# spkelle2/simple_mip_solver

Hardware: NVIDIA B200
Metric: node_lp_solves_per_sec (higher is better)
Workload: dtype f64

## Files before the change

### simple_mip_solver_b200/csrc/blp.cu

```cuda
#include "../../include/blp.h"

#include <cuda_runtime.h>
#include <dlfcn.h>

#include <cstdarg>
#include <cstdio>
#include <cstdlib>
#include <cstring>
#include <string>
#include <vector>

#include "blp_kernels.cuh"
#include "blp_prep.hpp"
#include "blp_simplex.cuh"

using namespace blp;

namespace {

thread_local std::string g_err;

int fail(int code, const char* fmt, ...) {
    char buf[512];
    va_list ap;
// ... 618 lines not shown
    return (o && o->max_active > 0 && o->max_active < B) ? o->max_active : B;
}

int blp_ld(int B) { return B <= 0 ? 0 : (B + kBlk - 1) / kBlk * kBlk; }

const char* blp_last_error(void) { return g_err.c_str(); }

const char* blp_version(void) {
#ifdef BLP_TUNING
    return "blp 0.2 sm_100a (tuning build: BLP_* environment variables are read)";
#else
    return "blp 0.2 sm_100a";
#endif
}

int blp_create(int device, int m, int n, int64_t nnz, const int32_t* rowptr, const int32_t* colidx,
               const double* val, const double* c, const double* row_lb, blp_handle* out) {
    if (!out) return fail(BLP_ERR_ARG, "blp_create: out is NULL");
    *out = nullptr;
    if (m < 1 || n < 1 || nnz < 0 || !rowptr || !c || !row_lb || (nnz > 0 && (!colidx || !val)))
        return fail(BLP_ERR_ARG, "blp_create: need m >= 1, n >= 1, nnz >= 0 and non-NULL arrays");
    if (rowptr[0] != 0 || rowptr[m] != nnz)
        return fail(BLP_ERR_ARG, "blp_create: rowptr[0] must be 0 and rowptr[m] must equal nnz");
    for (int i = 0; i < m; ++i) {
        if (rowptr[i + 1] < rowptr[i]) return fail(BLP_ERR_ARG, "blp_create: rowptr not monotone at row %d", i);
        if (!(std::fabs(row_lb[i]) < 1e30))
            return fail(BLP_ERR_ARG, "blp_create: row_lb[%d] is not finite (rows are 'a.x >= b')", i);
    }
    for (int64_t p = 0; p < nnz; ++p)
        if (colidx[p] < 0 || colidx[p] >= n || !std::isfinite(val[p]))
            return fail(BLP_ERR_ARG, "blp_create: entry %lld has column %d / non-finite value", (long long)p, colidx[p]);
    for (int j = 0; j < n; ++j)
        if (!std::isfinite(c[j])) return fail(BLP_ERR_ARG, "blp_create: c[%d] is not finite", j);
    int ndev = 0;
    CK(cudaGetDeviceCount(&ndev));
    if (device < 0 || device >= ndev)
        return fail(BLP_ERR_ARG, "blp_create: device %d out of range (%d visible)", device, ndev);
    CK(cudaSetDevice(device));
    blp_handle h = new (std::nothrow) blp_handle_s;
    if (!h) return fail(BLP_ERR_NOMEM, "blp_create: out of host memory");
    h->device = device;
    h->m_base = m;
    h->n = n;
    h->A0.rows = m;
    h->A0.cols = n;
    h->A0.ptr.assign(rowptr, rowptr + m + 1);
    h->A0.idx.assign(colidx, colidx + nnz);
    h->A0.val.assign(val, val + nnz);
    h->c0.assign(c, c + n);
    h->b0.assign(row_lb, row_lb + m);
    cudaDeviceGetAttribute(&h->num_sms, cudaDevAttrMultiProcessorCount, device);
    cudaDeviceGetAttribute(&h->coop_ok, cudaDevAttrCooperativeLaunch, device);
    cudaError_t e = cudaStreamCreateWithFlags(&h->stream, cudaStreamNonBlocking);
    if (e == cudaSuccess) e = cudaFuncSetAttribute(k_primal2<true>, cudaFuncAttributeMaxDynamicSharedMemorySize, 64 * 1024);
    if (e == cudaSuccess) e = cudaFuncSetAttribute(k_primal2<false>, cudaFuncAttributeMaxDynamicSharedMemorySize, 64 * 1024);
    if (e == cudaSuccess) e = cudaFuncSetAttribute(k_dual2<true>, cudaFuncAttributeMaxDynamicSharedMemorySize, 64 * 1024);
    if (e == cudaSuccess) e = cudaFuncSetAttribute(k_dual2<false>, cudaFuncAttributeMaxDynamicSharedMemorySize, 64 * 1024);
    if (e == cudaSuccess) e = cudaMallocHost(&h->h_counters, 16 * sizeof(int32_t));
    for (int q = 0; q < 4 && e == cudaSuccess; ++q) e = cudaEventCreate(&h->ev[q]);
    for (int q = 0; q < blp_handle_s::kLanes - 1 && e == cudaSuccess; ++q) {
        e = cudaStreamCreateWithFlags(&h->side[q], cudaStreamNonBlocking);
        if (e == cudaSuccess) e = cudaEventCreateWithFlags(&h->ev_join[q], cudaEventDisableTiming);
    }
    if (e == cudaSuccess) e = cudaEventCreateWithFlags(&h->ev_fork, cudaEventDisableTiming);
    if (e != cudaSuccess) {
        blp_destroy(h);
        return fail(BLP_ERR_CUDA, "blp_create: %s", cudaGetErrorString(e));
    }
    int rc = prepare(h);
    if (rc != BLP_OK) {
        blp_destroy(h);
        return rc;
    }
    *out = h;
    return BLP_OK;
}

int blp_append_rows(blp_handle h, int k, const int32_t* rowptr, const int32_t* colidx,
                    const double* val, const double* rhs, int* first_row_id) {
    if (!h) return fail(BLP_ERR_ARG, "blp_append_rows: NULL handle");
    if (k < 1 || !rowptr || !rhs) return fail(BLP_ERR_ARG, "blp_append_rows: need k >= 1 rows");
    if (rowptr[0] != 0) return fail(BLP_ERR_ARG, "blp_append_rows: rowptr[0] must be 0");
    const int64_t nnz = rowptr[k];
    for (int i = 0; i < k; ++i) {
        if (rowptr[i + 1] < rowptr[i]) return fail(BLP_ERR_ARG, "blp_append_rows: rowptr not monotone");
        if (!(std::fabs(rhs[i]) < 1e30)) return fail(BLP_ERR_ARG, "blp_append_rows: rhs[%d] not finite", i);
    }
    for (int64_t p = 0; p < nnz; ++p)
        if (colidx[p] < 0 || colidx[p] >= h->n || !std::isfinite(val[p]))
            return fail(BLP_ERR_ARG, "blp_append_rows: bad entry %lld", (long long)p);
    CK(cudaSetDevice(h->device));
    const int first = h->A0.rows;
    const int32_t base = h->A0.ptr.back();
    for (int i = 0; i < k; ++i) h->A0.ptr.push_back(base + rowptr[i + 1]);
    h->A0.idx.insert(h->A0.idx.end(), colidx, colidx + nnz);
    h->A0.val.insert(h->A0.val.end(), val, val + nnz);
    h->b0.insert(h->b0.end(), rhs, rhs + k);
    h->A0.rows += k;
    if (first_row_id) *first_row_id = first;
    return prepare(h);
}

int blp_truncate_rows(blp_handle h, int m_keep) {
    if (!h) return fail(BLP_ERR_ARG, "blp_truncate_rows: NULL handle");
    if (m_keep < h->m_base || m_keep > h->A0.rows)
        return fail(BLP_ERR_ARG, "blp_truncate_rows: m_keep %d outside [%d, %d]", m_keep, h->m_base, h->A0.rows);
    if (m_keep == h->A0.rows) return BLP_OK;
    CK(cudaSetDevice(h->device));
    h->A0.rows = m_keep;
    h->A0.ptr.resize(m_keep + 1);
// ... 70 lines not shown
    CK(cudaEventRecord(h->ev[0], st));
    CK(cudaMemsetAsync(S.counters, 0, 16 * sizeof(int32_t), st));
    if (freeze) CK(cudaMemsetAsync(cfrz_ws, 0, frz_bytes, st));
    if (have_mask)
        CK(cudaMemcpy2DAsync(mask_ws, S.ld, row_mask, ld_in, S.ld, P.m - P.m_base, cudaMemcpyDeviceToDevice, st));
    if (want_frac) {
        CK(cudaMemsetAsync(isint_ws, 0, P.n, st));
        k_set_isint<<<(n_int + 255) / 256, 256, 0, st>>>(int_idx, n_int, P.n, isint_ws);
        ++launches;
    }
    if (x) CK(cudaMemsetAsync(x, 0, (size_t)P.n * ld_in * sizeof(double), st));
    if (y) CK(cudaMemsetAsync(y, 0, (size_t)P.m * ld_in * sizeof(double), st));
    if (ld_in > B) {
        k_out_pad<<<(ld_in - B + 127) / 128, 128, 0, st>>>(O, B, ld_in);
        ++launches;
    }
    k_init_nodes<<<(S.ld + 127) / 128, 128, 0, st>>>(P, S);
    k_init_cols<<<elementwise_grid((size_t)P.n * S.ld), kCtaThreads, 0, st>>>(P, S, lb, ub, x0, ld_in);
    k_init_rows<<<elementwise_grid((size_t)P.m * S.ld), kCtaThreads, 0, st>>>(P, S, y0, ld_in);
    {
        Plan er0 = plan_rows(P.m, W, 1, kEvalChunks);
        er0.NT = NT;
        launch_check_rows(P, S, er0, 0, st);
    }
    k_build_lumask<<<elementwise_grid((size_t)P.n * (S.ld / 32) * 32), kCtaThreads, 0, st>>>(P, S);
    k_count_active<<<(W + 127) / 128, 128, 0, st>>>(S);
    launches += 6;
    CK(cudaGetLastError());
    CK(cudaMemcpyAsync(h->h_counters, S.counters, 13 * sizeof(int32_t), cudaMemcpyDeviceToHost, st));
    CK(cudaStreamSynchronize(st));
    int active = h->h_counters[0];

    auto make_plan = [&](int rows, int width, int rows_per_warp, int max_chunks) {
        Plan p = plan_rows(rows, width, rows_per_warp, max_chunks);
        const int pass = kWarps * (32 / NT);
        p.NT = NT;
        p.tiles = (width + NT - 1) / NT;
        int rpc = pass * std::max(rows_per_warp, 1);
        if (max_chunks > 0) {
            const int need = (rows + max_chunks - 1) / max_chunks;
            rpc = std::max(rpc, ((need + pass - 1) / pass) * pass);
        } else {
            while (rpc > 512 && rpc > pass) rpc -= pass;
        }
        p.rows_per_cta = rpc;
        p.chunks = std::max(1, (rows + rpc - 1) / rpc);
        return p;
    };
    const bool allow_v2 = env_int("BLP_V2", 1) != 0;
    const int graph_lanes = env_int("BLP_GRAPH_LANES", 2);
    const int rpw2 = std::min(env_int("BLP_ROWS_PER_WARP2", 16), kMaxChunkRows / kWarps);
    const int rpw2p = std::min(env_int("BLP_ROWS_PER_WARP2P", freeze ? 24 : rpw2), kMaxChunkRows / kWarps);
    auto step_plan = [&](int rows, int width, bool primal = false) {
        const bool v2 = allow_v2 && width >= kBlk && (long)std::max(P.n, P.m) * width >= (1L << 20);
        int r = v2 ? (primal ? rpw2p : rpw2) : rpw;
        Plan p = make_plan(rows, width, r, 0);
        auto shape = [&](Plan& q, int rr) {
            if (!v2) return;
            q.V = 2;
            q.tiles = (width + kBlk - 1) / kBlk;
            q.rows_per_cta = kWarps * std::max(rr, 1);
            q.chunks = std::max(1, (rows + q.rows_per_cta - 1) / q.rows_per_cta);
        };
        shape(p, r);
        while (r > 1 && (long)p.chunks * p.tiles < 148L * 12) {
            r /= 2;
            p = make_plan(rows, width, r, 0);
            shape(p, r);
        }
        return p;
    };
    Plan pc = step_plan(P.n, W, true), pr = step_plan(P.m, W);
    auto finish_step_plans = [&]() -> int {
        plan_chunks(pc, h->hptrAT, P.n, h->h_chunkC);
        plan_chunks(pr, h->hptrA, P.m, h->h_chunkR);
        CK(upload(h->chunkC, h->h_chunkC, st));
        CK(upload(h->chunkR, h->h_chunkR, st));
        pc.chunk_ptr = h->chunkC.as<int32_t>();
        pr.chunk_ptr = h->chunkR.as<int32_t>();
        return BLP_OK;
    };
    if ((rc = finish_step_plans()) != BLP_OK) return rc;
    Plan ec = make_plan(P.n, W, 1, kEvalChunks), er = make_plan(P.m, W, 1, kEvalChunks);
    D.chunksC = ec.chunks;
    D.chunksR = er.chunks;

    if (active < W) launch_harvest(P, S, O, ec, er, want_frac, st, &launches);

    int next = W, refills = 0;
    auto refill = [&]() -> int {
        while (next < B && active < S.B) {
            const int nnew = std::min(B - next, S.B - active);
            k_refill_plan<<<1, 1024, 0, st>>>(P, S, next, nnew);
            k_refill_cols<<<elementwise_grid((size_t)P.n * nnew), kCtaThreads, 0, st>>>(P, S, lb, ub, x0, ld_in, nnew);
            k_refill_rows<<<elementwise_grid((size_t)P.m * nnew), kCtaThreads, 0, st>>>(P, S, y0, row_mask, ld_in, nnew);
            launch_check_rows(P, S, er, 1, st);
            k_build_lumask<<<elementwise_grid((size_t)P.n * ((S.B + 31) / 32) * 32), kCtaThreads, 0, st>>>(P, S);
            k_count_active<<<(S.B + 127) / 128, 128, 0, st>>>(S);
            launches += 6;
            CK(cudaGetLastError());
            CK(cudaMemcpyAsync(h->h_counters, S.counters, 13 * sizeof(int32_t), cudaMemcpyDeviceToHost, st));
            CK(cudaStreamSynchronize(st));
            next += nnew;
            refills += nnew;
            active = h->h_counters[0];
            if (h->h_counters[3] > 0) launch_harvest(P, S, O, ec, er, want_frac, st, &launches);
        }
        return BLP_OK;
    };
    if ((rc = refill()) != BLP_OK) return rc;
    auto refreeze = [&](int mode) {
        if (!freeze || pc.V != 2) return;
        launches += launch_freeze(P, S, F, T, mode, st);
    };
    refreeze(2);

    const bool profile = o.profile == 1;
    const bool use_graph = o.use_graph && !profile;
    if (profile)
        while ((int)h->prof_ev.size() < 2 * 4 * K0 + 1) {
            cudaEvent_t e;
            CK(cudaEventCreate(&e));
            h->prof_ev.push_back(e);
        }

    bool coop = false;
    bool coop_rejected = false;
    const bool allow_coop = h->coop_ok && env_int("BLP_COOP", 1) != 0;
// ... 818 lines not shown
```

### simple_mip_solver_b200/csrc/blp_kernels.cuh

```cuda
#pragma once
#include <cstdint>
#include <cooperative_groups.h>
#include <cuda_runtime.h>

namespace blp {

#ifndef BLP_U
#define BLP_U 4
#endif
#ifndef BLP_MINB
#define BLP_MINB 6
#endif
#ifndef BLP_ANCHOR32
#define BLP_ANCHOR32 1
#endif
#if BLP_ANCHOR32
using anc_t = float;
using anc2_t = float2;
#else
using anc_t = double;
using anc2_t = double2;
#endif
constexpr int kCtaThreads = 256;
constexpr int kBlk = 64;
// ... 98 lines not shown
            const int4 e = __ldg(reinterpret_cast<const int4*>(ent + p));
            const double v = node_ok ? Vn[(size_t)e.x * ld] : 0.0;
            acc = fma(__hiloint2double(e.w, e.z), v, acc);
        }
    }
    return acc;
}

template <int NT>
__device__ __forceinline__ void row_dot_pair(const int32_t* __restrict__ ptr, const Ent* __restrict__ ent,
                                             int row, bool row_ok, const double* __restrict__ Vn,
                                             const double* __restrict__ Wn, bool node_ok, double& accv,
                                             double& accw) {
    constexpr int ld = kBlk;
    accv = 0.0;
    accw = 0.0;
    if (NT == 32 || (row_ok && node_ok)) {
        const int p0 = __ldg(ptr + row), p1 = __ldg(ptr + row + 1);
        for (int p = p0; p < p1; p += 4) {
            int4 e[4];
            double v[4], w[4];
#pragma unroll
            for (int q = 0; q < 4; ++q) {
                v[q] = 0.0;
                w[q] = 0.0;
                e[q] = make_int4(0, 0, 0, 0);
                if (p + q < p1) {
                    e[q] = __ldg(reinterpret_cast<const int4*>(ent + p + q));
                    if (node_ok) {
                        v[q] = Vn[(size_t)e[q].x * ld];
                        w[q] = Wn[(size_t)e[q].x * ld];
                    }
                }
            }
#pragma unroll
            for (int q = 0; q < 4; ++q) {
                const double cf = __hiloint2double(e[q].w, e[q].z);
                accv = fma(cf, v[q], accv);
                accw = fma(cf, w[q], accw);
            }
        }
    }
}

struct Slab {
    const int* sp;
    const int4* se;
    int base;
    const int* ends = nullptr;
};

extern __shared__ int4 dyn_smem[];

__device__ __forceinline__ Slab stage_slab(const int32_t* __restrict__ ptr,
                                           const Ent* __restrict__ ent, const int r0, const int r1,
                                           const int rows_per_cta, const int cap,
                                           int4* const smem_base = dyn_smem) {
    int* sp = reinterpret_cast<int*>(smem_base);
    int4* se = smem_base + (rows_per_cta + 4) / 4;
    const int nrows = r1 - r0;
    for (int t = threadIdx.x; t <= nrows; t += kCtaThreads) sp[t] = __ldg(ptr + r0 + t);
    __syncthreads();
    Slab s;
    s.sp = sp;
    s.base = sp[0];
    s.se = nullptr;
    const int cnt = sp[nrows] - s.base;
    if (cnt <= cap) {
        const int4* __restrict__ src = reinterpret_cast<const int4*>(ent) + s.base;
        for (int t = threadIdx.x; t < cnt; t += kCtaThreads) se[t] = __ldg(src + t);
        __syncthreads();
        s.se = se;
    }
    return s;
}

template <bool SHARED>
__device__ __forceinline__ double dot_entries(const int4* __restrict__ E, const int p0, const int p1,
                                              const double* __restrict__ Vn, const int ld,
                                              const bool node_ok) {
    constexpr int kU = BLP_U;
    double acc = 0.0;
    for (int p = p0; p < p1; p += kU) {
        double v[kU];
#pragma unroll
        for (int q = 0; q < kU; ++q) {
            v[q] = 0.0;
            if (p + q < p1) {
                const int col = SHARED ? E[p + q].x : __ldg(&E[p + q].x);
                if (node_ok) v[q] = Vn[(size_t)col * ld];
            }
        }
#pragma unroll
        for (int q = 0; q < kU; ++q)
            if (p + q < p1) {
                const int2 c = SHARED ? *reinterpret_cast<const int2*>(&E[p + q].z)
                                      : __ldg(reinterpret_cast<const int2*>(&E[p + q].z));
                acc = fma(__hiloint2double(c.y, c.x), v[q], acc);
            }
    }
    return acc;
}

template <int NT>
__device__ __forceinline__ double slab_dot(const Slab& sl, const Ent* __restrict__ ent, const int lr,
                                           const bool row_ok, const double* __restrict__ Vn,
                                           const int ld, const bool node_ok) {
    if (NT != 32 && !(row_ok && node_ok)) return 0.0;
    const int p0 = sl.sp[lr], p1 = sl.sp[lr + 1];
    if (sl.se) return dot_entries<true>(sl.se - sl.base, p0, p1, Vn, ld, node_ok);
    return dot_entries<false>(reinterpret_cast<const int4*>(ent), p0, p1, Vn, ld, node_ok);
}

constexpr int kLongRow = 96;
// ... 158 lines not shown
    dual_chunk<NT, MAJOR>(P, S, it, rows_per_cta, cap, chunk_ptr, blockIdx.x, blockIdx.y);
}

struct CoopPlan {
    int rpcC, capC, nchC, rpcR, capR, nchR, tiles;
    const int* chunkC;
    const int* chunkR;
};

template <int NT>
__global__ void __launch_bounds__(kCtaThreads, 4)
k_period_coop(const DevProb P, const DevState S, const int K, const CoopPlan C) {
    cooperative_groups::grid_group grid = cooperative_groups::this_grid();
    const int w = blockIdx.x;
    const bool hasC = w < C.nchC * C.tiles, hasR = w < C.nchR * C.tiles;
    const int cxC = w % C.nchC, cyC = w / C.nchC, cxR = w % C.nchR, cyR = w / C.nchR;
    Slab slC{nullptr, nullptr, 0}, slR{nullptr, nullptr, 0};
    int4* const baseR = dyn_smem + (C.rpcC + 4) / 4 + C.capC;
    if (hasC) slC = stage_slab(P.cptr, P.cent, __ldg(C.chunkC + 2 * cxC), __ldg(C.chunkC + 2 * cxC + 1), C.rpcC, C.capC);
    if (hasR) slR = stage_slab(P.rowptr, P.ent, __ldg(C.chunkR + 2 * cxR), __ldg(C.chunkR + 2 * cxR + 1), C.rpcR, C.capR, baseR);
    for (int it = 0; it < K; ++it) {
        const bool major = it == K - 1;
        if (hasC) {
            if (major) primal_chunk<NT, true>(P, S, it, C.rpcC, C.capC, C.chunkC, cxC, cyC, &slC);
            else primal_chunk<NT, false>(P, S, it, C.rpcC, C.capC, C.chunkC, cxC, cyC, &slC);
        }
        grid.sync();
        if (hasR) {
            if (major) dual_chunk<NT, true>(P, S, it, C.rpcR, C.capR, C.chunkR, cxR, cyR, &slR);
            else dual_chunk<NT, false>(P, S, it, C.rpcR, C.capR, C.chunkR, cxR, cyR, &slR);
        }
        grid.sync();
    }
}

#ifndef BLP_MINB2
#define BLP_MINB2 5
#endif

__device__ __forceinline__ double2 ld2(const double* p) { return *reinterpret_cast<const double2*>(p); }
__device__ __forceinline__ double2 ldcs2(const double* p) {
    return __ldcs(reinterpret_cast<const double2*>(p));
}
__device__ __forceinline__ double2 ldcs2(const float* p) {
    const float2 v = __ldcs(reinterpret_cast<const float2*>(p));
    return make_double2((double)v.x, (double)v.y);
}
__device__ __forceinline__ void st2(double* p, const double2 v, const bool k0, const bool k1) {
    if (k0 && k1) *reinterpret_cast<double2*>(p) = v;
    else if (k0) p[0] = v.x;
    else if (k1) p[1] = v.y;
}

template <bool SHARED>
__device__ __forceinline__ void dot2_entries(const int4* __restrict__ E, const int p0, const int p1,
                                             const double* __restrict__ Vn, double& g0, double& g1,
                                             const int ld = kBlk) {
    constexpr int kU = BLP_U;
    for (int p = p0; p < p1; p += kU) {
        double2 v[kU];
#pragma unroll
        for (int q = 0; q < kU; ++q) {
            v[q] = make_double2(0.0, 0.0);
            if (p + q < p1) {
                const int col = SHARED ? E[p + q].x : __ldg(&E[p + q].x);
                v[q] = ld2(Vn + (size_t)col * ld);
            }
        }
#pragma unroll
        for (int q = 0; q < kU; ++q)
            if (p + q < p1) {
                const int2 c = SHARED ? *reinterpret_cast<const int2*>(&E[p + q].z)
                                      : __ldg(reinterpret_cast<const int2*>(&E[p + q].z));
                const double cf = __hiloint2double(c.y, c.x);
                g0 = fma(cf, v[q].x, g0);
                g1 = fma(cf, v[q].y, g1);
            }
    }
}

__device__ __forceinline__ void slab_dot2(const Slab& sl, const Ent* __restrict__ ent, const int lr,
                                          const double* __restrict__ Vn, double& g0, double& g1,
                                          const int ld = kBlk) {
    const int p0 = sl.sp[lr], p1 = sl.ends ? sl.ends[lr] : sl.sp[lr + 1];
    if (sl.se) dot2_entries<true>(sl.se - sl.base, p0, p1, Vn, g0, g1, ld);
    else dot2_entries<false>(reinterpret_cast<const int4*>(ent), p0, p1, Vn, g0, g1, ld);
}


__device__ __forceinline__ void coop_dot2(const Slab& sl, const Ent* __restrict__ ent,
                                          const double* __restrict__ Vn, const int warp, const int lane,
                                          double& g0, double& g1) {
    __shared__ double2 red[kWarps][32];
    const int p0 = sl.sp[0], p1 = sl.ends ? sl.ends[0] : sl.sp[1];
    const int seg = ((p1 - p0 + kWarps - 1) / kWarps + BLP_U - 1) / BLP_U * BLP_U;
    const int a = min(p1, p0 + warp * seg), b = min(p1, a + seg);
    double s0 = 0.0, s1 = 0.0;
    if (sl.se) dot2_entries<true>(sl.se - sl.base, a, b, Vn, s0, s1);
    else dot2_entries<false>(reinterpret_cast<const int4*>(ent), a, b, Vn, s0, s1);
    red[warp][lane] = make_double2(s0, s1);
    __syncthreads();
    g0 = 0.0;
    g1 = 0.0;
#pragma unroll
    for (int w = 0; w < kWarps; ++w) {
        g0 += red[w][lane].x;
        g1 += red[w][lane].y;
    }
}

template <bool SHARED>
__device__ __forceinline__ void dot2_entries_pair(const int4* __restrict__ E, int pa, const int pa1, int pb,
                                                  const int pb1, const double* __restrict__ Vn, double& ga0,
                                                  double& ga1, double& gb0, double& gb1) {
    constexpr int kU = BLP_U;
    while (pa < pa1 || pb < pb1) {
        double2 va[kU], vb[kU];
#pragma unroll
        for (int q = 0; q < kU; ++q) {
            va[q] = make_double2(0.0, 0.0);
            if (pa + q < pa1) {
                const int col = SHARED ? E[pa + q].x : __ldg(&E[pa + q].x);
                va[q] = ld2(Vn + (size_t)col * kBlk);
            }
        }
#pragma unroll
        for (int q = 0; q < kU; ++q) {
            vb[q] = make_double2(0.0, 0.0);
            if (pb + q < pb1) {
                const int col = SHARED ? E[pb + q].x : __ldg(&E[pb + q].x);
                vb[q] = ld2(Vn + (size_t)col * kBlk);
            }
        }
#pragma unroll
        for (int q = 0; q < kU; ++q)
            if (pa + q < pa1) {
                const int2 c = SHARED ? *reinterpret_cast<const int2*>(&E[pa + q].z)
                                      : __ldg(reinterpret_cast<const int2*>(&E[pa + q].z));
                const double cf = __hiloint2double(c.y, c.x);
                ga0 = fma(cf, va[q].x, ga0);
                ga1 = fma(cf, va[q].y, ga1);
            }
#pragma unroll
        for (int q = 0; q < kU; ++q)
            if (pb + q < pb1) {
                const int2 c = SHARED ? *reinterpret_cast<const int2*>(&E[pb + q].z)
                                      : __ldg(reinterpret_cast<const int2*>(&E[pb + q].z));
                const double cf = __hiloint2double(c.y, c.x);
                gb0 = fma(cf, vb[q].x, gb0);
                gb1 = fma(cf, vb[q].y, gb1);
            }
        pa += kU;
        pb += kU;
    }
}

constexpr int kMaxChunkRows = 512;
__shared__ uint16_t s_rows[kMaxChunkRows];
__shared__ int s_ends[kMaxChunkRows];
__shared__ int s_group[kMaxChunkRows / 32 + 1];
__shared__ int s_nrows;

__device__ __forceinline__ Slab stage_slab_frozen(const int32_t* __restrict__ ptr, const Ent* __restrict__ ent,
                                                  const int32_t* __restrict__ ends, const uint8_t* __restrict__ flags,
                                                  const int rows, const int h0, const unsigned live, const int r0,
                                                  const int r1, const int rows_per_cta, const int cap) {
    int* sp = reinterpret_cast<int*>(dyn_smem);
    int4* se = dyn_smem + (rows_per_cta + 4) / 4;
    const int nrows = r1 - r0, lane = threadIdx.x & 31;
    const bool live0 = (live & 0x0000ffffu) != 0, live1 = (live & 0xffff0000u) != 0;
    const uint8_t* __restrict__ f0 = flags + (size_t)h0 * rows + r0;
    const uint8_t* __restrict__ f1 = f0 + rows;
    bool keep[2];
    int rank[2];
#pragma unroll
    for (int q = 0; q < 2; ++q) {
        const int t = threadIdx.x + q * kCtaThreads;
        keep[q] = false;
        if (t <= nrows) sp[t] = __ldg(ptr + r0 + t);
        if (t < nrows) {
            s_ends[t] = __ldg(ends + r0 + t);
            keep[q] = !((!live0 || f0[t] != 0) && (!live1 || f1[t] != 0));
        }
        const unsigned bal = __ballot_sync(0xffffffffu, keep[q]);
        rank[q] = __popc(bal & ((1u << lane) - 1u));
        if (lane == 0) s_group[t >> 5] = __popc(bal);
    }
    __syncthreads();
    Slab s;
    s.sp = sp;
    s.base = sp[0];
    s.se = nullptr;
    s.ends = s_ends;
    const int cnt = sp[nrows] - s.base;
    if (cnt <= cap) {
        const int4* __restrict__ src = reinterpret_cast<const int4*>(ent) + s.base;
        for (int t = threadIdx.x; t < cnt; t += kCtaThreads) se[t] = __ldg(src + t);
        s.se = se;
    }
    const int groups = (nrows + 31) >> 5;
#pragma unroll
    for (int q = 0; q < 2; ++q) {
        const int t = threadIdx.x + q * kCtaThreads;
        if (keep[q]) {
            int before = 0;
            for (int g = 0; g < (t >> 5); ++g) before += s_group[g];
            s_rows[before + rank[q]] = (uint16_t)t;
        }
    }
    if (threadIdx.x == 0) {
        int total = 0;
        for (int g = 0; g < groups; ++g) total += s_group[g];
        s_nrows = total;
    }
    __syncthreads();
    return s;
}

#ifndef BLP_PAIR_ROWS
#define BLP_PAIR_ROWS 0
#endif
#ifndef BLP_PAIR_ROWS_DUAL
#define BLP_PAIR_ROWS_DUAL 0
#endif
#ifndef BLP_MINB2P
#define BLP_MINB2P 4
#endif

template <bool MAJOR>
__global__ void __launch_bounds__(kCtaThreads, BLP_PAIR_ROWS ? BLP_MINB2P : BLP_MINB2)
k_primal2(const DevProb P, const DevState S, const int it, const int rows_per_cta, const int cap,
          const int* __restrict__ chunk_ptr, const int tile0) {
    const int lane = threadIdx.x & 31, warp = threadIdx.x >> 5;
    const int node = (tile0 + blockIdx.y) * kBlk + lane * 2;
    const bool k0 = node < S.B && S.fin[node] == 0;
    const bool k1 = node + 1 < S.B && S.fin[node + 1] == 0;
    const unsigned live = __ballot_sync(0xffffffffu, k0 || k1);
    if (live == 0) return;
    double w0 = 0, w1 = 0, tau0 = 0, tau1 = 0;
    if (k0) {
        const int s = S.sbase[node] + it;
        w0 = (double)s / (double)(s + 1);
        tau0 = S.eta[node] / S.omega[node];
    }
    if (k1) {
        const int s = S.sbase[node + 1] + it;
        w1 = (double)s / (double)(s + 1);
        tau1 = S.eta[node + 1] / S.omega[node + 1];
    }
    const int r0 = __ldg(chunk_ptr + 2 * blockIdx.x);
    const int r1 = __ldg(chunk_ptr + 2 * blockIdx.x + 1);
    const bool frz = !MAJOR && S.cfrz != nullptr;
    const int tile = tile0 + blockIdx.y;
    const Ent* __restrict__ cent = frz ? S.fentAT + (size_t)tile * P.nnz : P.cent;
    const Slab sl = frz ? stage_slab_frozen(P.cptr, cent, S.fendAT + (size_t)tile * P.n, S.cfrz, P.n, tile * 2, live,
                                            r0, r1, rows_per_cta, cap)
                        : stage_slab(P.cptr, P.cent, r0, r1, rows_per_cta, cap);
    const size_t base = tix(0, node, P.n);
    const double* __restrict__ yn = S.y + tix(0, node, P.m);
    const size_t fblk = (size_t)(node >> 5) * P.n;
    const unsigned bit = node & 31;
    const bool coop = (r1 - r0 == 1) && (sl.sp[1] - sl.sp[0] > kLongRow);
    double cg0 = 0.0, cg1 = 0.0;
    if (coop) {
        if (frz && s_nrows == 0) return;
        coop_dot2(sl, cent, yn, warp, lane, cg0, cg1);
        if (warp != 0) return;
    }
#if BLP_PAIR_ROWS
    if (!coop && !frz) {
        for (int j = r0 + warp; j < r1; j += 2 * kWarps) {
            const int jb = j + kWarps;
            const bool hb = jb < r1;
            const size_t ea = base + (size_t)j * kBlk, eb = base + (size_t)(hb ? jb : j) * kBlk;
            const double2 xba = ld2(S.xbar + ea), xbb = ld2(S.xbar + eb);
            const double2 aa = ldcs2(S.xa + ea), ab = ldcs2(S.xa + eb);
            const int jb_ = hb ? jb : j;
            const uint32_t mka = (__ldg(S.lumask + fblk + j) >> bit) & 3u;
            const uint32_t mkb = (__ldg(S.lumask + fblk + jb_) >> bit) & 3u;
            double loa0 = __ldg(S.lref + fblk + j), hia0 = __ldg(S.uref + fblk + j);
            double lob0 = __ldg(S.lref + fblk + jb_), hib0 = __ldg(S.uref + fblk + jb_);
            double loa1 = loa0, hia1 = hia0, lob1 = lob0, hib1 = hib0;
            if (mka) {
                const double2 l2 = ldcs2(S.l + ea), u2 = ldcs2(S.u + ea);
                if (mka & 1u) { loa0 = l2.x; hia0 = u2.x; }
                if (mka & 2u) { loa1 = l2.y; hia1 = u2.y; }
            }
            if (mkb) {
                const double2 l2 = ldcs2(S.l + eb), u2 = ldcs2(S.u + eb);
                if (mkb & 1u) { lob0 = l2.x; hib0 = u2.x; }
                if (mkb & 2u) { lob1 = l2.y; hib1 = u2.y; }
            }
            double ga0 = 0.0, ga1 = 0.0, gb0 = 0.0, gb1 = 0.0;
            {
                const int pa = sl.sp[j - r0], pa1 = sl.sp[j - r0 + 1];
                const int pb = hb ? sl.sp[jb - r0] : 0, pb1 = hb ? sl.sp[jb - r0 + 1] : 0;
                if (sl.se) dot2_entries_pair<true>(sl.se - sl.base, pa, pa1, pb, pb1, yn, ga0, ga1, gb0, gb1);
                else dot2_entries_pair<false>(reinterpret_cast<const int4*>(P.cent), pa, pa1, pb, pb1, yn, ga0, ga1, gb0, gb1);
            }
            {
                const double cj = __ldg(P.c + j);
                const double xc0 = fma(w0, xba.x - aa.x, aa.x), xc1 = fma(w1, xba.y - aa.y, aa.y);
                const double xp0 = fmin(fmax(xc0 - tau0 * (cj - ga0), loa0), hia0);
                const double xp1 = fmin(fmax(xc1 - tau1 * (cj - ga1), loa1), hia1);
                st2(S.xbar + ea, make_double2(2.0 * xp0 - xc0, 2.0 * xp1 - xc1), k0, k1);
                if constexpr (MAJOR) {
                    st2(S.X1 + ea, make_double2(xp0, xp1), k0, k1);
                    st2(S.DX + ea, make_double2(xp0 - xc0, xp1 - xc1), k0, k1);
                    st2(S.G + ea, make_double2(ga0, ga1), k0, k1);
                }
            }
            if (hb) {
                const double cj = __ldg(P.c + jb);
                const double xc0 = fma(w0, xbb.x - ab.x, ab.x), xc1 = fma(w1, xbb.y - ab.y, ab.y);
                const double xp0 = fmin(fmax(xc0 - tau0 * (cj - gb0), lob0), hib0);
                const double xp1 = fmin(fmax(xc1 - tau1 * (cj - gb1), lob1), hib1);
                st2(S.xbar + eb, make_double2(2.0 * xp0 - xc0, 2.0 * xp1 - xc1), k0, k1);
                if constexpr (MAJOR) {
                    st2(S.X1 + eb, make_double2(xp0, xp1), k0, k1);
                    st2(S.DX + eb, make_double2(xp0 - xc0, xp1 - xc1), k0, k1);
                    st2(S.G + eb, make_double2(gb0, gb1), k0, k1);
                }
            }
        }
        return;
    }
#endif
    const int ntrips = frz ? s_nrows : r1 - r0;
    for (int k = warp; k < ntrips; k += kWarps) {
        const int j = r0 + (frz ? (int)s_rows[k] : k);
        const size_t e = base + (size_t)j * kBlk;
        const double2 xb = ld2(S.xbar + e);
        const double2 a = ldcs2(S.xa + e);
        const uint32_t mk = (__ldg(S.lumask + fblk + j) >> bit) & 3u;
        double lo0 = __ldg(S.lref + fblk + j), hi0 = __ldg(S.uref + fblk + j);
        double lo1 = lo0, hi1 = hi0;
        if (mk) {
            const double2 l2 = ldcs2(S.l + e), u2 = ldcs2(S.u + e);
            if (mk & 1u) { lo0 = l2.x; hi0 = u2.x; }
            if (mk & 2u) { lo1 = l2.y; hi1 = u2.y; }
        }
        double g0 = cg0, g1 = cg1;
        if (!coop) slab_dot2(sl, cent, j - r0, yn, g0, g1);
        const double cj = __ldg(P.c + j);
        const double xc0 = fma(w0, xb.x - a.x, a.x), xc1 = fma(w1, xb.y - a.y, a.y);
        const double xp0 = fmin(fmax(xc0 - tau0 * (cj - g0), lo0), hi0);
        const double xp1 = fmin(fmax(xc1 - tau1 * (cj - g1), lo1), hi1);
        st2(S.xbar + e, make_double2(2.0 * xp0 - xc0, 2.0 * xp1 - xc1), k0, k1);
        if constexpr (MAJOR) {
            st2(S.X1 + e, make_double2(xp0, xp1), k0, k1);
            st2(S.DX + e, make_double2(xp0 - xc0, xp1 - xc1), k0, k1);
            st2(S.G + e, make_double2(g0, g1), k0, k1);
        }
    }
}

template <bool MAJOR>
__global__ void __launch_bounds__(kCtaThreads, BLP_PAIR_ROWS_DUAL ? BLP_MINB2P : BLP_MINB2)
k_dual2(const DevProb P, const DevState S, const int it, const int rows_per_cta, const int cap,
        const int* __restrict__ chunk_ptr, const int tile0) {
    const int lane = threadIdx.x & 31, warp = threadIdx.x >> 5;
    const int node = (tile0 + blockIdx.y) * kBlk + lane * 2;
    const bool k0 = node < S.B && S.fin[node] == 0;
    const bool k1 = node + 1 < S.B && S.fin[node + 1] == 0;
    const unsigned live = __ballot_sync(0xffffffffu, k0 || k1);
    if (live == 0) return;
    double w0 = 0, w1 = 0, sig0 = 0, sig1 = 0;
    if (k0) {
        const int s = S.sbase[node] + it;
        w0 = (double)(s + 1) / (double)(s + 2);
        sig0 = S.eta[node] * S.omega[node];
    }
    if (k1) {
        const int s = S.sbase[node + 1] + it;
        w1 = (double)(s + 1) / (double)(s + 2);
        sig1 = S.eta[node + 1] * S.omega[node + 1];
    }
    const int r0 = __ldg(chunk_ptr + 2 * blockIdx.x);
    const int r1 = __ldg(chunk_ptr + 2 * blockIdx.x + 1);
    const bool frz = !MAJOR && S.rfrz != nullptr;
    const int tile = tile0 + blockIdx.y;
    const Ent* __restrict__ aent = frz ? S.fentA + (size_t)tile * P.nnz : P.ent;
    const double* __restrict__ rconst = S.rconst + (size_t)tile * P.m;
    const Slab sl = frz ? stage_slab_frozen(P.rowptr, aent, S.fendA + (size_t)tile * P.m, S.rfrz, P.m, tile * 2, live,
                                            r0, r1, rows_per_cta, cap)
                        : stage_slab(P.rowptr, P.ent, r0, r1, rows_per_cta, cap);
    const size_t base = tix(0, node, P.m);
    const double* __restrict__ xn = S.xbar + tix(0, node, P.n);
    const bool coop = (r1 - r0 == 1) && (sl.sp[1] - sl.sp[0] > kLongRow);
    double cg0 = 0.0, cg1 = 0.0;
    if (coop) {
        if (frz && s_nrows == 0) return;
        coop_dot2(sl, aent, xn, warp, lane, cg0, cg1);
        if (warp != 0) return;
        if (frz) {
            const double rc = __ldg(rconst + r0);
            cg0 += rc;
            cg1 += rc;
        }
    }
#if BLP_PAIR_ROWS_DUAL
    if (!coop && !frz) {
        for (int i = r0 + warp; i < r1; i += 2 * kWarps) {
            const int ib = i + kWarps;
            const bool hb = ib < r1;
            const int ib_ = hb ? ib : i;
            const size_t ea = base + (size_t)i * kBlk, eb = base + (size_t)ib_ * kBlk;
            const double2 yca = ld2(S.y + ea), ycb = ld2(S.y + eb);
            const double2 aa = ldcs2(S.ya + ea), ab = ldcs2(S.ya + eb);
            bool ona0 = true, ona1 = true, onb0 = true, onb1 = true;
            if (S.rowmask) {
                if (i >= P.m_base) {
                    const uint8_t* mrow = S.rowmask + (size_t)(i - P.m_base) * S.ld + node;
                    ona0 = mrow[0] != 0;
                    ona1 = mrow[1] != 0;
                }
                if (ib_ >= P.m_base) {
                    const uint8_t* mrow = S.rowmask + (size_t)(ib_ - P.m_base) * S.ld + node;
                    onb0 = mrow[0] != 0;
                    onb1 = mrow[1] != 0;
                }
            }
            double axa0 = 0.0, axa1 = 0.0, axb0 = 0.0, axb1 = 0.0;
            {
                const int pa = sl.sp[i - r0], pa1 = sl.sp[i - r0 + 1];
                const int pb = hb ? sl.sp[ib - r0] : 0, pb1 = hb ? sl.sp[ib - r0 + 1] : 0;
                if (sl.se) dot2_entries_pair<true>(sl.se - sl.base, pa, pa1, pb, pb1, xn, axa0, axa1, axb0, axb1);
                else dot2_entries_pair<false>(reinterpret_cast<const int4*>(P.ent), pa, pa1, pb, pb1, xn, axa0, axa1, axb0, axb1);
            }
            {
                const double bi = __ldg(P.b + i);
                const double yp0 = ona0 ? fmax(0.0, yca.x + sig0 * (bi - axa0)) : 0.0;
                const double yp1 = ona1 ? fmax(0.0, yca.y + sig1 * (bi - axa1)) : 0.0;
                st2(S.y + ea, make_double2(fma(w0, (2.0 * yp0 - yca.x) - aa.x, aa.x),
                                           fma(w1, (2.0 * yp1 - yca.y) - aa.y, aa.y)), k0, k1);
                if constexpr (MAJOR) {
                    st2(S.Y1 + ea, make_double2(yp0, yp1), k0, k1);
                    st2(S.DY + ea, make_double2(yp0 - yca.x, yp1 - yca.y), k0, k1);
                }
            }
            if (hb) {
                const double bi = __ldg(P.b + ib);
                const double yp0 = onb0 ? fmax(0.0, ycb.x + sig0 * (bi - axb0)) : 0.0;
                const double yp1 = onb1 ? fmax(0.0, ycb.y + sig1 * (bi - axb1)) : 0.0;
                st2(S.y + eb, make_double2(fma(w0, (2.0 * yp0 - ycb.x) - ab.x, ab.x),
                                           fma(w1, (2.0 * yp1 - ycb.y) - ab.y, ab.y)), k0, k1);
                if constexpr (MAJOR) {
                    st2(S.Y1 + eb, make_double2(yp0, yp1), k0, k1);
                    st2(S.DY + eb, make_double2(yp0 - ycb.x, yp1 - ycb.y), k0, k1);
                }
            }
        }
        return;
    }
#endif
    const int ntrips = frz ? s_nrows : r1 - r0;
    for (int k = warp; k < ntrips; k += kWarps) {
        const int i = r0 + (frz ? (int)s_rows[k] : k);
        const size_t e = base + (size_t)i * kBlk;
        const double2 yc = ld2(S.y + e);
        const double2 a = ldcs2(S.ya + e);
        bool on0 = true, on1 = true;
        if (i >= P.m_base && S.rowmask) {
            const uint8_t* mrow = S.rowmask + (size_t)(i - P.m_base) * S.ld + node;
            on0 = mrow[0] != 0;
            on1 = mrow[1] != 0;
        }
        double ax0 = cg0, ax1 = cg1;
        if (!coop) {
            if (frz) ax0 = ax1 = __ldg(rconst + i);
            slab_dot2(sl, aent, i - r0, xn, ax0, ax1);
        }
        const double bi = __ldg(P.b + i);
        const double yp0 = on0 ? fmax(0.0, yc.x + sig0 * (bi - ax0)) : 0.0;
        const double yp1 = on1 ? fmax(0.0, yc.y + sig1 * (bi - ax1)) : 0.0;
        st2(S.y + e, make_double2(fma(w0, (2.0 * yp0 - yc.x) - a.x, a.x),
                                  fma(w1, (2.0 * yp1 - yc.y) - a.y, a.y)), k0, k1);
        if constexpr (MAJOR) {
            st2(S.Y1 + e, make_double2(yp0, yp1), k0, k1);
            st2(S.DY + e, make_double2(yp0 - yc.x, yp1 - yc.y), k0, k1);
        }
    }
}


template <int NT, int NACC, int NSUM>
__device__ __forceinline__ void cta_reduce_store(double (&acc)[NACC], double* __restrict__ part,
                                                 int ld, int node_base) {
    __shared__ double sm[NACC][kCtaThreads];
#pragma unroll
    for (int a = 0; a < NACC; ++a) sm[a][threadIdx.x] = acc[a];
    __syncthreads();
    for (int t = threadIdx.x; t < NT * NACC; t += kCtaThreads) {
        const int a = t / NT, nl = t % NT;
        double r = sm[a][nl];
        for (int q = nl + NT; q < kCtaThreads; q += NT)
            r = (a < NSUM) ? r + sm[a][q] : fmax(r, sm[a][q]);
        part[((size_t)blockIdx.x * NACC + a) * ld + node_base + nl] = r;
    }
}

template <int NT>
__global__ void __launch_bounds__(kCtaThreads)
k_eval_cols(const DevProb P, const DevState S, const int rows_per_cta) {
    constexpr int RW = 32 / NT;
    const int lane = threadIdx.x & 31, warp = threadIdx.x >> 5;
    const int node = blockIdx.y * NT + (lane % NT);
    const int sub = lane / NT;
    const bool node_ok = node < S.B && S.fin[node] == 0;
    if (__ballot_sync(0xffffffffu, node_ok) == 0) return;
    double acc[C_N];
#pragma unroll
    for (int a = 0; a < C_N; ++a) acc[a] = 0.0;
    const int r0 = blockIdx.x * rows_per_cta;
    const int r1 = min(P.n, r0 + rows_per_cta);
    for (int jb = r0 + warp * RW; jb < r1; jb += kWarps * RW) {
        const int j = jb + sub;
        const bool row_ok = j < r1;
        const size_t e = tix(j, node, P.n);
        const double gp = row_dot<NT>(P.cptr, P.cent, row_ok ? j : 0, row_ok, S.Y1 + tix(0, node, P.m),
                                      node_ok && row_ok);
        if (row_ok && node_ok) {
            const double xp = S.X1[e], dx = S.DX[e], g = S.G[e];
            const double lo = S.l[e], hi = S.u[e], xa = (double)S.xa[e];
            const double cj = __ldg(P.c + j), cs = __ldg(P.colscale + j);
            const bool fl = !is_inf(lo), fu = !is_inf(hi);
            acc[C_DX2] = fma(dx, dx, acc[C_DX2]);
            acc[C_CROSS] = fma(dx, gp - g, acc[C_CROSS]);
            const double r = cj - gp;
            const double lam = (r > 0.0) ? (fl ? r : 0.0) : (fu ? r : 0.0);
            const double dres = (r - lam) * cs;
            acc[C_DRES2] = fma(dres, dres, acc[C_DRES2]);
            acc[C_CX] = fma(cj, xp, acc[C_CX]);
            if (lam > 0.0) acc[C_BND] = fma(lo, lam, acc[C_BND]);
// ... 1011 lines not shown
```

Measured before the change: 159.7.

## Stage per-row scalars in shared memory and use 32-bit indexing in v2 kernels

The v2 primal and dual kernels now copy per-row scalars (c, lref/uref, lumask, b, rconst) into extra dynamic shared memory while the slab is staged, and read them from there inside the row loop. Per-node weights and step sizes go to shared arrays. Index arithmetic switches to unsigned 32-bit offsets, with v2 gated on the index range fitting in 32 bits. The dot product loop gets specialised shared and global paths that skip zero padding. This aims to cut redundant global loads and 64-bit address math, at the cost of more shared memory per CTA (raised to 72KB), which may lower occupancy.

```diff
diff --git a/simple_mip_solver_b200/csrc/blp.cu b/simple_mip_solver_b200/csrc/blp.cu
--- a/simple_mip_solver_b200/csrc/blp.cu
+++ b/simple_mip_solver_b200/csrc/blp.cu
@@ -694,10 +694,10 @@
     cudaDeviceGetAttribute(&h->num_sms, cudaDevAttrMultiProcessorCount, device);
     cudaDeviceGetAttribute(&h->coop_ok, cudaDevAttrCooperativeLaunch, device);
     cudaError_t e = cudaStreamCreateWithFlags(&h->stream, cudaStreamNonBlocking);
-    if (e == cudaSuccess) e = cudaFuncSetAttribute(k_primal2<true>, cudaFuncAttributeMaxDynamicSharedMemorySize, 64 * 1024);
-    if (e == cudaSuccess) e = cudaFuncSetAttribute(k_primal2<false>, cudaFuncAttributeMaxDynamicSharedMemorySize, 64 * 1024);
-    if (e == cudaSuccess) e = cudaFuncSetAttribute(k_dual2<true>, cudaFuncAttributeMaxDynamicSharedMemorySize, 64 * 1024);
-    if (e == cudaSuccess) e = cudaFuncSetAttribute(k_dual2<false>, cudaFuncAttributeMaxDynamicSharedMemorySize, 64 * 1024);
+    if (e == cudaSuccess) e = cudaFuncSetAttribute(k_primal2<true>, cudaFuncAttributeMaxDynamicSharedMemorySize, 72 * 1024);
+    if (e == cudaSuccess) e = cudaFuncSetAttribute(k_primal2<false>, cudaFuncAttributeMaxDynamicSharedMemorySize, 72 * 1024);
+    if (e == cudaSuccess) e = cudaFuncSetAttribute(k_dual2<true>, cudaFuncAttributeMaxDynamicSharedMemorySize, 72 * 1024);
+    if (e == cudaSuccess) e = cudaFuncSetAttribute(k_dual2<false>, cudaFuncAttributeMaxDynamicSharedMemorySize, 72 * 1024);
     if (e == cudaSuccess) e = cudaMallocHost(&h->h_counters, 16 * sizeof(int32_t));
     for (int q = 0; q < 4 && e == cudaSuccess; ++q) e = cudaEventCreate(&h->ev[q]);
     for (int q = 0; q < blp_handle_s::kLanes - 1 && e == cudaSuccess; ++q) {
@@ -874,7 +874,8 @@
     const int rpw2 = std::min(env_int("BLP_ROWS_PER_WARP2", 16), kMaxChunkRows / kWarps);
     const int rpw2p = std::min(env_int("BLP_ROWS_PER_WARP2P", freeze ? 24 : rpw2), kMaxChunkRows / kWarps);
     auto step_plan = [&](int rows, int width, bool primal = false) {
-        const bool v2 = allow_v2 && width >= kBlk && (long)std::max(P.n, P.m) * width >= (1L << 20);
+        const bool v2 = allow_v2 && width >= kBlk && (long)std::max(P.n, P.m) * width >= (1L << 20) &&
+                        (size_t)std::max(P.n, P.m) * S.ld < ((size_t)1 << 32);
         int r = v2 ? (primal ? rpw2p : rpw2) : rpw;
         Plan p = make_plan(rows, width, r, 0);
         auto shape = [&](Plan& q, int rr) {
@@ -896,6 +897,10 @@
     auto finish_step_plans = [&]() -> int {
         plan_chunks(pc, h->hptrAT, P.n, h->h_chunkC);
         plan_chunks(pr, h->hptrA, P.m, h->h_chunkR);
+        if (pc.V == 2) {
+            pc.smem += (size_t)kPrimalRowBytes * pc.rows_per_cta;
+            pr.smem += (size_t)kDualRowBytes * pr.rows_per_cta;
+        }
         CK(upload(h->chunkC, h->h_chunkC, st));
         CK(upload(h->chunkR, h->h_chunkR, st));
         pc.chunk_ptr = h->chunkC.as<int32_t>();
diff --git a/simple_mip_solver_b200/csrc/blp_kernels.cuh b/simple_mip_solver_b200/csrc/blp_kernels.cuh
--- a/simple_mip_solver_b200/csrc/blp_kernels.cuh
+++ b/simple_mip_solver_b200/csrc/blp_kernels.cuh
@@ -174,14 +174,22 @@
 
 extern __shared__ int4 dyn_smem[];
 
+struct NoRowScalars {
+    __device__ __forceinline__ void operator()(int, int) const {}
+};
+
+template <class RS = NoRowScalars>
 __device__ __forceinline__ Slab stage_slab(const int32_t* __restrict__ ptr,
                                            const Ent* __restrict__ ent, const int r0, const int r1,
                                            const int rows_per_cta, const int cap,
-                                           int4* const smem_base = dyn_smem) {
+                                           int4* const smem_base = dyn_smem, const RS rs = RS()) {
     int* sp = reinterpret_cast<int*>(smem_base);
     int4* se = smem_base + (rows_per_cta + 4) / 4;
     const int nrows = r1 - r0;
-    for (int t = threadIdx.x; t <= nrows; t += kCtaThreads) sp[t] = __ldg(ptr + r0 + t);
+    for (int t = threadIdx.x; t <= nrows; t += kCtaThreads) {
+        sp[t] = __ldg(ptr + r0 + t);
+        if (t < nrows) rs(r0 + t, t);
+    }
     __syncthreads();
     Slab s;
     s.sp = sp;
@@ -446,19 +454,20 @@
     else if (k1) p[1] = v.y;
 }
 
-template <bool SHARED>
+template <bool SHARED, class I = size_t, bool PAD = true>
 __device__ __forceinline__ void dot2_entries(const int4* __restrict__ E, const int p0, const int p1,
                                              const double* __restrict__ Vn, double& g0, double& g1,
-                                             const int ld = kBlk) {
+                                             const int ld = kBlk, const I off = 0) {
     constexpr int kU = BLP_U;
+#pragma unroll 1
     for (int p = p0; p < p1; p += kU) {
         double2 v[kU];
 #pragma unroll
         for (int q = 0; q < kU; ++q) {
-            v[q] = make_double2(0.0, 0.0);
+            if (PAD) v[q] = make_double2(0.0, 0.0);
             if (p + q < p1) {
                 const int col = SHARED ? E[p + q].x : __ldg(&E[p + q].x);
-                v[q] = ld2(Vn + (size_t)col * ld);
+                v[q] = ld2(Vn + (off + (I)col * (I)ld));
             }
         }
 #pragma unroll
@@ -555,10 +564,11 @@
 __shared__ int s_group[kMaxChunkRows / 32 + 1];
 __shared__ int s_nrows;
 
+template <class RS>
 __device__ __forceinline__ Slab stage_slab_frozen(const int32_t* __restrict__ ptr, const Ent* __restrict__ ent,
                                                   const int32_t* __restrict__ ends, const uint8_t* __restrict__ flags,
                                                   const int rows, const int h0, const unsigned live, const int r0,
-                                                  const int r1, const int rows_per_cta, const int cap) {
+                                                  const int r1, const int rows_per_cta, const int cap, const RS rs) {
     int* sp = reinterpret_cast<int*>(dyn_smem);
     int4* se = dyn_smem + (rows_per_cta + 4) / 4;
     const int nrows = r1 - r0, lane = threadIdx.x & 31;
@@ -600,6 +610,7 @@
             int before = 0;
             for (int g = 0; g < (t >> 5); ++g) before += s_group[g];
             s_rows[before + rank[q]] = (uint16_t)t;
+            rs(r0 + t, before + rank[q]);
         }
     }
     if (threadIdx.x == 0) {
@@ -620,6 +631,57 @@
 #ifndef BLP_MINB2P
 #define BLP_MINB2P 4
 #endif
+
+__shared__ double2 s_wv[32], s_sv[32];
+
+__device__ __forceinline__ int4* row_scalar_smem(const int rows_per_cta, const int cap) {
+    return dyn_smem + (rows_per_cta + 4) / 4 + cap;
+}
+constexpr int kPrimalRowBytes = 48, kDualRowBytes = 16;
+
+struct PrimalRowScalars {
+    const double* c; const double* lref; const double* uref; const uint32_t* lumask;
+    size_t rows;
+    struct View {
+        double2* lu; double* cs; uint32_t* mk;
+        __device__ __forceinline__ View(const int rows_per_cta, const int cap) {
+            lu = reinterpret_cast<double2*>(row_scalar_smem(rows_per_cta, cap));
+            cs = reinterpret_cast<double*>(lu + 2 * rows_per_cta);
+            mk = reinterpret_cast<uint32_t*>(cs + rows_per_cta);
+        }
+    };
+    View v;
+    __device__ PrimalRowScalars(const DevProb& P, const DevState& S, const int h0, const int rows_per_cta,
+                                const int cap) : v(rows_per_cta, cap) {
+        const size_t f = (size_t)h0 * P.n;
+        c = P.c; lref = S.lref + f; uref = S.uref + f; lumask = S.lumask + f; rows = P.n;
+    }
+    __device__ __forceinline__ void operator()(const int j, const int slot) const {
+        v.cs[slot] = __ldg(c + j);
+        v.lu[2 * slot] = make_double2(__ldg(lref + j), __ldg(uref + j));
+        v.lu[2 * slot + 1] = make_double2(__ldg(lref + rows + j), __ldg(uref + rows + j));
+        v.mk[2 * slot] = __ldg(lumask + j);
+        v.mk[2 * slot + 1] = __ldg(lumask + rows + j);
+    }
+};
+
+struct DualRowScalars {
+    const double* b; const double* rc;
+    struct View {
+        double* bs; double* rcs;
+        __device__ __forceinline__ View(const int rows_per_cta, const int cap) {
+            bs = reinterpret_cast<double*>(row_scalar_smem(rows_per_cta, cap));
+            rcs = bs + rows_per_cta;
+        }
+    };
+    View v;
+    __device__ DualRowScalars(const DevProb& P, const double* rconst, const int rows_per_cta, const int cap)
+        : b(P.b), rc(rconst), v(rows_per_cta, cap) {}
+    __device__ __forceinline__ void operator()(const int i, const int slot) const {
+        v.bs[slot] = __ldg(b + i);
+        v.rcs[slot] = rc ? __ldg(rc + i) : 0.0;
+    }
+};
 
 template <bool MAJOR>
 __global__ void __launch_bounds__(kCtaThreads, BLP_PAIR_ROWS ? BLP_MINB2P : BLP_MINB2)
@@ -631,6 +693,9 @@
     const bool k1 = node + 1 < S.B && S.fin[node + 1] == 0;
     const unsigned live = __ballot_sync(0xffffffffu, k0 || k1);
     if (live == 0) return;
+    const unsigned run0 = __ballot_sync(0xffffffffu, k0), run1 = __ballot_sync(0xffffffffu, k1);
+    auto st0 = [&] { return MAJOR ? k0 : ((run0 >> (threadIdx.x & 31)) & 1u) != 0; };
+    auto st1 = [&] { return MAJOR ? k1 : ((run1 >> (threadIdx.x & 31)) & 1u) != 0; };
     double w0 = 0, w1 = 0, tau0 = 0, tau1 = 0;
     if (k0) {
         const int s = S.sbase[node] + it;
@@ -642,18 +707,27 @@
         w1 = (double)s / (double)(s + 1);
         tau1 = S.eta[node + 1] / S.omega[node + 1];
     }
+    if (warp == 0) {
+        s_wv[lane] = make_double2(w0, w1);
+        s_sv[lane] = make_double2(tau0, tau1);
+    }
     const int r0 = __ldg(chunk_ptr + 2 * blockIdx.x);
     const int r1 = __ldg(chunk_ptr + 2 * blockIdx.x + 1);
     const bool frz = !MAJOR && S.cfrz != nullptr;
     const int tile = tile0 + blockIdx.y;
     const Ent* __restrict__ cent = frz ? S.fentAT + (size_t)tile * P.nnz : P.cent;
+    const PrimalRowScalars rs(P, S, tile * 2, rows_per_cta, cap);
     const Slab sl = frz ? stage_slab_frozen(P.cptr, cent, S.fendAT + (size_t)tile * P.n, S.cfrz, P.n, tile * 2, live,
-                                            r0, r1, rows_per_cta, cap)
-                        : stage_slab(P.cptr, P.cent, r0, r1, rows_per_cta, cap);
-    const size_t base = tix(0, node, P.n);
+                                            r0, r1, rows_per_cta, cap, rs)
+                        : stage_slab(P.cptr, P.cent, r0, r1, rows_per_cta, cap, dyn_smem, rs);
+    const unsigned base = (unsigned)tix(0, node, P.n);
     const double* __restrict__ yn = S.y + tix(0, node, P.m);
+    const unsigned yoff = (unsigned)tix(0, node, P.m);
+#if BLP_PAIR_ROWS
     const size_t fblk = (size_t)(node >> 5) * P.n;
+#endif
     const unsigned bit = node & 31;
+    const int half = lane >> 4;
     const bool coop = (r1 - r0 == 1) && (sl.sp[1] - sl.sp[0] > kLongRow);
     double cg0 = 0.0, cg1 = 0.0;
     if (coop) {
@@ -720,32 +794,53 @@
         return;
     }
 #endif
-    const int ntrips = frz ? s_nrows : r1 - r0;
-    for (int k = warp; k < ntrips; k += kWarps) {
-        const int j = r0 + (frz ? (int)s_rows[k] : k);
-        const size_t e = base + (size_t)j * kBlk;
+    auto trip = [&](const int k, double g0, double g1, auto gather) {
+        const int lr = frz ? (int)s_rows[k] : k;
+        const unsigned e = base + (unsigned)(r0 + lr) * kBlk;
         const double2 xb = ld2(S.xbar + e);
         const double2 a = ldcs2(S.xa + e);
-        const uint32_t mk = (__ldg(S.lumask + fblk + j) >> bit) & 3u;
-        double lo0 = __ldg(S.lref + fblk + j), hi0 = __ldg(S.uref + fblk + j);
-        double lo1 = lo0, hi1 = hi0;
-        if (mk) {
-            const double2 l2 = ldcs2(S.l + e), u2 = ldcs2(S.u + e);
-            if (mk & 1u) { lo0 = l2.x; hi0 = u2.x; }
-            if (mk & 2u) { lo1 = l2.y; hi1 = u2.y; }
-        }
-        double g0 = cg0, g1 = cg1;
-        if (!coop) slab_dot2(sl, cent, j - r0, yn, g0, g1);
-        const double cj = __ldg(P.c + j);
-        const double xc0 = fma(w0, xb.x - a.x, a.x), xc1 = fma(w1, xb.y - a.y, a.y);
-        const double xp0 = fmin(fmax(xc0 - tau0 * (cj - g0), lo0), hi0);
-        const double xp1 = fmin(fmax(xc1 - tau1 * (cj - g1), lo1), hi1);
-        st2(S.xbar + e, make_double2(2.0 * xp0 - xc0, 2.0 * xp1 - xc1), k0, k1);
+        gather(lr, g0, g1);
+        const PrimalRowScalars::View rv(rows_per_cta, cap);
+        const uint32_t mk = (rv.mk[2 * k + half] >> bit) & 3u;
+        const double2 lh = rv.lu[2 * k + half];
+        double lo0 = lh.x, hi0 = lh.y, lo1 = lh.x, hi1 = lh.y;
+        if (mk & 1u) {
+            lo0 = __ldcs(S.l + e);
+            hi0 = __ldcs(S.u + e);
+        }
+        if (mk & 2u) {
+            lo1 = __ldcs(S.l + e + 1);
+            hi1 = __ldcs(S.u + e + 1);
+        }
+        const double cj = rv.cs[k];
+        const double2 w = s_wv[lane], tau = s_sv[lane];
+        const double xc0 = fma(w.x, xb.x - a.x, a.x), xc1 = fma(w.y, xb.y - a.y, a.y);
+        const double xp0 = fmin(fmax(xc0 - tau.x * (cj - g0), lo0), hi0);
+        const double xp1 = fmin(fmax(xc1 - tau.y * (cj - g1), lo1), hi1);
+        st2(S.xbar + e, make_double2(2.0 * xp0 - xc0, 2.0 * xp1 - xc1), st0(), st1());
         if constexpr (MAJOR) {
-            st2(S.X1 + e, make_double2(xp0, xp1), k0, k1);
-            st2(S.DX + e, make_double2(xp0 - xc0, xp1 - xc1), k0, k1);
-            st2(S.G + e, make_double2(g0, g1), k0, k1);
-        }
+            st2(S.X1 + e, make_double2(xp0, xp1), st0(), st1());
+            st2(S.DX + e, make_double2(xp0 - xc0, xp1 - xc1), st0(), st1());
+            st2(S.G + e, make_double2(g0, g1), st0(), st1());
+        }
+    };
+    if (coop) {
+        trip(0, cg0, cg1, [](int, double&, double&) {});
+        return;
+    }
+    const int ntrips = frz ? s_nrows : r1 - r0;
+    if (sl.se) {
+        const int4* const E = sl.se - sl.base;
+        for (int k = warp; k < ntrips; k += kWarps)
+            trip(k, 0.0, 0.0, [&](const int lr, double& g0, double& g1) {
+                dot2_entries<true, unsigned, false>(E, sl.sp[lr], frz ? s_ends[lr] : sl.sp[lr + 1], S.y, g0, g1, kBlk, yoff);
+            });
+    } else {
+        const int4* const E = reinterpret_cast<const int4*>(cent);
+        for (int k = warp; k < ntrips; k += kWarps)
+            trip(k, 0.0, 0.0, [&](const int lr, double& g0, double& g1) {
+                dot2_entries<false, unsigned, false>(E, sl.sp[lr], frz ? s_ends[lr] : sl.sp[lr + 1], S.y, g0, g1, kBlk, yoff);
+            });
     }
 }
 
@@ -759,6 +854,9 @@
     const bool k1 = node + 1 < S.B && S.fin[node + 1] == 0;
     const unsigned live = __ballot_sync(0xffffffffu, k0 || k1);
     if (live == 0) return;
+    const unsigned run0 = __ballot_sync(0xffffffffu, k0), run1 = __ballot_sync(0xffffffffu, k1);
+    auto st0 = [&] { return ((run0 >> (threadIdx.x & 31)) & 1u) != 0; };
+    auto st1 = [&] { return ((run1 >> (threadIdx.x & 31)) & 1u) != 0; };
     double w0 = 0, w1 = 0, sig0 = 0, sig1 = 0;
     if (k0) {
         const int s = S.sbase[node] + it;
@@ -769,6 +867,10 @@
         const int s = S.sbase[node + 1] + it;
         w1 = (double)(s + 1) / (double)(s + 2);
         sig1 = S.eta[node + 1] * S.omega[node + 1];
+    }
+    if (warp == 0) {
+        s_wv[lane] = make_double2(w0, w1);
+        s_sv[lane] = make_double2(sig0, sig1);
     }
     const int r0 = __ldg(chunk_ptr + 2 * blockIdx.x);
     const int r1 = __ldg(chunk_ptr + 2 * blockIdx.x + 1);
@@ -776,11 +878,13 @@
     const int tile = tile0 + blockIdx.y;
     const Ent* __restrict__ aent = frz ? S.fentA + (size_t)tile * P.nnz : P.ent;
     const double* __restrict__ rconst = S.rconst + (size_t)tile * P.m;
+    const DualRowScalars rs(P, frz ? rconst : nullptr, rows_per_cta, cap);
     const Slab sl = frz ? stage_slab_frozen(P.rowptr, aent, S.fendA + (size_t)tile * P.m, S.rfrz, P.m, tile * 2, live,
-                                            r0, r1, rows_per_cta, cap)
-                        : stage_slab(P.rowptr, P.ent, r0, r1, rows_per_cta, cap);
-    const size_t base = tix(0, node, P.m);
+                                            r0, r1, rows_per_cta, cap, rs)
+                        : stage_slab(P.rowptr, P.ent, r0, r1, rows_per_cta, cap, dyn_smem, rs);
+    const unsigned base = (unsigned)tix(0, node, P.m);
     const double* __restrict__ xn = S.xbar + tix(0, node, P.n);
+    const unsigned xoff = (unsigned)tix(0, node, P.n);
     const bool coop = (r1 - r0 == 1) && (sl.sp[1] - sl.sp[0] > kLongRow);
     double cg0 = 0.0, cg1 = 0.0;
     if (coop) {
@@ -848,10 +952,10 @@
         return;
     }
 #endif
-    const int ntrips = frz ? s_nrows : r1 - r0;
-    for (int k = warp; k < ntrips; k += kWarps) {
-        const int i = r0 + (frz ? (int)s_rows[k] : k);
-        const size_t e = base + (size_t)i * kBlk;
+    auto trip = [&](const int k, auto gather) {
+        const int lr = frz ? (int)s_rows[k] : k;
+        const int i = r0 + lr;
+        const unsigned e = base + (unsigned)i * kBlk;
         const double2 yc = ld2(S.y + e);
         const double2 a = ldcs2(S.ya + e);
         bool on0 = true, on1 = true;
@@ -860,20 +964,38 @@
             on0 = mrow[0] != 0;
             on1 = mrow[1] != 0;
         }
-        double ax0 = cg0, ax1 = cg1;
-        if (!coop) {
-            if (frz) ax0 = ax1 = __ldg(rconst + i);
-            slab_dot2(sl, aent, i - r0, xn, ax0, ax1);
-        }
-        const double bi = __ldg(P.b + i);
-        const double yp0 = on0 ? fmax(0.0, yc.x + sig0 * (bi - ax0)) : 0.0;
-        const double yp1 = on1 ? fmax(0.0, yc.y + sig1 * (bi - ax1)) : 0.0;
-        st2(S.y + e, make_double2(fma(w0, (2.0 * yp0 - yc.x) - a.x, a.x),
-                                  fma(w1, (2.0 * yp1 - yc.y) - a.y, a.y)), k0, k1);
+        double ax0, ax1;
+        gather(k, lr, ax0, ax1);
+        const double bi = DualRowScalars::View(rows_per_cta, cap).bs[k];
+        const double2 w = s_wv[lane], sig = s_sv[lane];
+        const double yp0 = on0 ? fmax(0.0, yc.x + sig.x * (bi - ax0)) : 0.0;
+        const double yp1 = on1 ? fmax(0.0, yc.y + sig.y * (bi - ax1)) : 0.0;
+        st2(S.y + e, make_double2(fma(w.x, (2.0 * yp0 - yc.x) - a.x, a.x),
+                                  fma(w.y, (2.0 * yp1 - yc.y) - a.y, a.y)), st0(), st1());
         if constexpr (MAJOR) {
-            st2(S.Y1 + e, make_double2(yp0, yp1), k0, k1);
-            st2(S.DY + e, make_double2(yp0 - yc.x, yp1 - yc.y), k0, k1);
-        }
+            st2(S.Y1 + e, make_double2(yp0, yp1), st0(), st1());
+            st2(S.DY + e, make_double2(yp0 - yc.x, yp1 - yc.y), st0(), st1());
+        }
+    };
+    if (coop) {
+        trip(0, [&](int, int, double& ax0, double& ax1) { ax0 = cg0; ax1 = cg1; });
+        return;
+    }
+    const int ntrips = frz ? s_nrows : r1 - r0;
+    if (sl.se) {
+        const int4* const E = sl.se - sl.base;
+        for (int k = warp; k < ntrips; k += kWarps)
+            trip(k, [&](const int k_, const int lr, double& ax0, double& ax1) {
+                ax0 = ax1 = DualRowScalars::View(rows_per_cta, cap).rcs[k_];
+                dot2_entries<true, unsigned, false>(E, sl.sp[lr], frz ? s_ends[lr] : sl.sp[lr + 1], S.xbar, ax0, ax1, kBlk, xoff);
+            });
+    } else {
+        const int4* const E = reinterpret_cast<const int4*>(aent);
+        for (int k = warp; k < ntrips; k += kWarps)
+            trip(k, [&](const int k_, const int lr, double& ax0, double& ax1) {
+                ax0 = ax1 = DualRowScalars::View(rows_per_cta, cap).rcs[k_];
+                dot2_entries<false, unsigned, false>(E, sl.sp[lr], frz ? s_ends[lr] : sl.sp[lr + 1], S.xbar, ax0, ax1, kBlk, xoff);
+            });
     }
 }
 
```

New measurement: 174.4 (median of 6 runs). 9.2% higher.
